# andrew-sha/CUDAFluidSimulator

Measured on AMD Instinct MI355X. Metric: particle-steps/sec (first 41 of the 100 steps of -m time), higher is better.
Workload: dtype f32

## Files before the change

### cudafluidsimulator_amd/csrc/sweep_common.h

```cpp
#pragma once
#include "sph_device.h"

#define SW_THREADS 256
#define SW_WAVES (SW_THREADS / SPH_WAVE)
#ifndef SW_UNROLL
#define SW_UNROLL 4
#endif
#ifndef SW_CAP
#define SW_CAP 384
#endif
#ifndef SW_QCAP
#define SW_QCAP 32
#endif

__device__ __forceinline__ int3 sweep_cell(const DevParams &P, float x, float y,
                                           float z) {
    int3 c;
    c.x = min(max((int)(x / P.h), 0), P.D - 1);
    c.y = min(max((int)(y / P.h), 0), P.D - 1);
    c.z = min(max((int)(z / P.h), 0), P.D - 1);
    return c;
}

__device__ __forceinline__ void load_runs(const DevParams &P,
                                          const int2 *__restrict__ cellRange,
                                          int3 c, bool valid, int (&js)[9],
                                          int (&je)[9]) {
    const int x0 = max(c.x - 1, 0), x1 = min(c.x + 1, P.D - 1);
    const int xm = min(x0 + 1, x1);
    int2 r0[9], r1[9], r2[9];
#pragma unroll
    for (int r = 0; r < 9; ++r) {
        const int sz = min(max(c.z + (r / 3 - 1), 0), P.D - 1);
        const int sy = min(max(c.y + (r % 3 - 1), 0), P.D - 1);
        const int base = sy * P.D + sz * P.D * P.D;
        r0[r] = cellRange[base + x0];
        r1[r] = cellRange[base + xm];
        r2[r] = cellRange[base + x1];
    }
#pragma unroll
    for (int r = 0; r < 9; ++r) {
        const int sz = c.z + (r / 3 - 1), sy = c.y + (r % 3 - 1);
        const bool inGrid = valid && sy >= 0 && sy < P.D && sz >= 0 && sz < P.D;
        const bool n0 = r0[r].y > r0[r].x, n1 = r1[r].y > r1[r].x, n2 = r2[r].y > r2[r].x;
        const bool any = inGrid && (n0 | n1 | n2);
        const int s = n0 ? r0[r].x : (n1 ? r1[r].x : r2[r].x);
        const int e = n2 ? r2[r].y : (n1 ? r1[r].y : r0[r].y);
        js[r] = any ? s : 0;
        je[r] = any ? e : 0;
    }
}


__device__ __forceinline__ void density_pair(const DevParams &P, float pix, float piy,
                                             float piz, float4 pj, float &rho) {
    float dx = pix - pj.x;
    float dy = piy - pj.y;
    float dz = piz - pj.z;
    float dist2 = dx * dx + dy * dy + dz * dz;
    if (!(dist2 > P.h2)) {
        float diff = P.h2 - dist2;
        rho += SPH_MASS * (P.dcoef * diff * diff * diff);
    }
}

struct ForceAcc {
    float fx, fy, fz;
};

__device__ __forceinline__ float sw_recip_refined(float b) {
    const float r0 = __builtin_amdgcn_rcpf(b);
    const float e0 = __builtin_fmaf(-b, r0, 1.0f);
    return __builtin_fmaf(e0, r0, r0);
}
__device__ __forceinline__ float sw_div_with(float a, float b, float r1) {
    const float q0 = a * r1;
    const float e1 = __builtin_fmaf(-b, q0, a);
    const float q1 = __builtin_fmaf(e1, r1, q0);
    const float e2 = __builtin_fmaf(-b, q1, a);
    return __builtin_fmaf(e2, r1, q1);
}
__device__ __forceinline__ float sw_sqrt(float x) {
    const float s = __builtin_amdgcn_sqrtf(x);
    const float sm = __int_as_float(__float_as_int(s) - 1);
    const float sp = __int_as_float(__float_as_int(s) + 1);
    const float tm = __builtin_fmaf(-sm, s, x);
    const float tp = __builtin_fmaf(-sp, s, x);
    float r = (0.f >= tm) ? sm : s;
    r = (0.f < tp) ? sp : r;
    return r;
}

template <bool SLIM>
__device__ __forceinline__ void force_pair(const DevParams &P, float pix, float piy,
                                           float piz, float vix, float viy, float viz,
                                           float prs_i, float4 pj, float4 vj,
                                           ForceAcc &F) {
    float dx = pix - pj.x;
    float dy = piy - pj.y;
    float dz = piz - pj.z;
    float dist2 = dx * dx + dy * dy + dz * dz;
    float rho_j = vj.w;
    float prs_j = fmaxf(0.f, SPH_GAS_CONSTANT * (rho_j - SPH_REST_DENSITY));
    if constexpr (SLIM) {
        const float dist = sw_sqrt(dist2);
        const bool tiny = dist < SPH_EPS_F;
        const bool inP = !(dist2 > P.h2) && !tiny, inV = !(dist > P.h) && !tiny;
        const float rrho = sw_recip_refined(rho_j);
        const float hd = P.h - dist;
        const float fPressure = 0.5f * sw_div_with(-SPH_MASS * (prs_i + prs_j), rho_j, rrho);
        const float scale = sw_div_with((-P.vcoef) * hd * hd, dist, sw_recip_refined(dist));
        const float fViscosity = sw_div_with(SPH_VISCOSITY * SPH_MASS * (P.vcoef * hd), rho_j, rrho);
        const float scaleG = inP ? scale : 0.f, fViscG = inV ? fViscosity : 0.f;
        float kx = dx * scaleG, ky = dy * scaleG, kz = dz * scaleG;
        kx *= fPressure;
        ky *= fPressure;
        kz *= fPressure;
        float dvx = vj.x - vix, dvy = vj.y - viy, dvz = vj.z - viz;
        dvx *= fViscG;
        dvy *= fViscG;
        dvz *= fViscG;
        F.fx += kx;
        F.fy += ky;
        F.fz += kz;
        F.fx += dvx;
        F.fy += dvy;
        F.fz += dvz;
    } else {
        float dist = sqrtf(dist2);
        bool tiny = dist < SPH_EPS_F;
        if (!(dist2 > P.h2) && !tiny) {
            float fPressure = -SPH_MASS * (prs_i + prs_j) / (2.f * rho_j);
            float scale = (-P.vcoef) * (P.h - dist) * (P.h - dist) / dist;
            float kx = dx * scale, ky = dy * scale, kz = dz * scale;
            kx *= fPressure;
            ky *= fPressure;
            kz *= fPressure;
            F.fx += kx;
            F.fy += ky;
            F.fz += kz;
        }
        if (!(dist > P.h) && !tiny) {
            float fViscosity =
                SPH_VISCOSITY * SPH_MASS * (P.vcoef * (P.h - dist)) / rho_j;
            float dvx = vj.x - vix, dvy = vj.y - viy, dvz = vj.z - viz;
            dvx *= fViscosity;
            dvy *= fViscosity;
            dvz *= fViscosity;
            F.fx += dvx;
            F.fy += dvy;
            F.fz += dvz;
        }
    }
}

__device__ __forceinline__ float fast_dist2(float pix, float piy, float piz, float4 pj,
                                            float &dx, float &dy, float &dz) {
    dx = pix - pj.x;
    dy = piy - pj.y;
    dz = piz - pj.z;
    return __builtin_fmaf(dz, dz, __builtin_fmaf(dy, dy, dx * dx));
}

__device__ __forceinline__ void force_pair_fast(const DevParams &P, float pix, float piy,
                                                float piz, float vix, float viy, float viz,
                                                float prs_i, float4 pj, float4 vj,
                                                ForceAcc &F) {
    float dx, dy, dz;
    const float dist2 = fast_dist2(pix, piy, piz, pj, dx, dy, dz);
    const float rho_j = vj.w;
    const float inv_rho = __builtin_amdgcn_rcpf(rho_j);
    const float prs_j = fmaxf(0.f, rho_j - SPH_REST_DENSITY);
    const float inv_dist = __builtin_amdgcn_rsqf(dist2);
    const float dist = dist2 * inv_dist;
    const bool ok = !(dist2 > P.h2) && !(dist < SPH_EPS_F) && dist2 > 0.f;
    if (ok) {
        const float hd = P.h - dist;
        const float s = (0.5f * SPH_MASS * P.vcoef) * (prs_i + prs_j) * inv_rho * (hd * hd) * inv_dist;
        const float fv = (SPH_VISCOSITY * SPH_MASS * P.vcoef) * hd * inv_rho;
        F.fx = __builtin_fmaf(vj.x - vix, fv, __builtin_fmaf(dx, s, F.fx));
        F.fy = __builtin_fmaf(vj.y - viy, fv, __builtin_fmaf(dy, s, F.fy));
        F.fz = __builtin_fmaf(vj.z - viz, fv, __builtin_fmaf(dz, s, F.fz));
    }
}

__device__ __forceinline__ void integrate_particle(const DevParams &P, float4 &p,
                                                   float &vx, float &vy, float &vz,
                                                   const ForceAcc &F, float density) {
    const float timestep = P.dt;
    vx += timestep * F.fx / density;
    vy += timestep * (F.fy / density + SPH_GRAVITY);
    vz += timestep * F.fz / density;

    p.x += timestep * vx;
    p.y += timestep * vy;
    p.z += timestep * vz;

    if (p.x < P.h) { p.x = P.h; vx *= -SPH_ELASTICITY; }
    else if (p.x > P.boxHi) { p.x = P.boxHi; vx *= -SPH_ELASTICITY; }
    if (p.y < P.h) { p.y = P.h; vy *= -SPH_ELASTICITY; }
    else if (p.y > P.boxHi) { p.y = P.boxHi; vy *= -SPH_ELASTICITY; }
    if (p.z < P.h) { p.z = P.h; vz *= -SPH_ELASTICITY; }
    else if (p.z > P.boxHi) { p.z = P.boxHi; vz *= -SPH_ELASTICITY; }

    if (fabsf(vx) < SPH_EPS_F) vx = 0;
    if (fabsf(vy) < SPH_EPS_F) vy = 0;
    if (fabsf(vz) < SPH_EPS_F) vz = 0;
}

__device__ __forceinline__ void store_particle(const SweepArgs &A, int i, float4 p,
                                               float vx, float vy, float vz,
                                               float rho, const ForceAcc &F) {
    A.pos_out[i] = p;
    A.vel_out[i] = make_float4(vx, vy, vz, rho);
    if (A.host_order_pos) {
        uint32_t id = __float_as_uint(p.w);
        float *o = A.host_order_pos + 3 * (size_t)id;
        o[0] = p.x;
        o[1] = p.y;
        o[2] = p.z;
    }
    if (A.force_out) A.force_out[i] = make_float4(F.fx, F.fy, F.fz, 0.f);
}

__device__ __forceinline__ int xcd_tile(int b, int nb, int C, int rot = 0) {
    int base = 0, R = nb, r = b;
    if (C > 0) {
        const int G = 8 * C;
        const int ng = nb / G, g = b / G;
        if (g < ng) {
            r = b - g * G;
            const int x = rot > 0 ? ((r & 7) + g / rot) & 7 : (r & 7);
            return g * G + x * C + (r >> 3);
        }
        base = ng * G;
        R = nb - base;
        r = b - base;
    }
    const int xcd = r & 7, idx = r >> 3;
    const int q = R >> 3, rem = R & 7;
    return base + xcd * q + min(xcd, rem) + idx;
}

__device__ __forceinline__ uint32_t wave_sum_u32(uint32_t v) {
#pragma unroll
    for (int off = 32; off > 0; off >>= 1) v += __shfl_xor(v, off);
    return v;
}
```

### cudafluidsimulator_amd/csrc/sweeps_list.hip

```cpp
#include "sweep_common.h"

#define SL_NONE 0xFFFFFFFFu

#ifndef SL_WINDOW
#define SL_WINDOW 160
#endif
#ifndef SL_K1_THREADS
#define SL_K1_THREADS 64
#endif

#ifndef SL_K1_WAVES
#define SL_K1_WAVES 6
#endif
__device__ __forceinline__ void sl_store_quiet(const SweepArgs &A, int i, bool valid, float rho, int lane) {
    const unsigned long long calm = A.calm[(i - lane) >> 6];
    const float prs = fmaxf(0.f, SPH_GAS_CONSTANT * (rho - SPH_REST_DENSITY));
    const bool q = valid && prs == 0.f && ((calm >> lane) & 1ull);
    const unsigned long long qb = __ballot(q), vb = __ballot(valid);
    if (lane == 0) {
        reinterpret_cast<unsigned long long *>(A.quiet)[(i - lane) >> 6] = qb;
        if (A.quietAll && qb != vb) *A.quietAll = 0u;
    }
}
__device__ __forceinline__ uint32_t sl_quiet_window(const uint32_t *__restrict__ quiet, uint32_t j) {
    const uint32_t lo = quiet[j >> 5], hi = quiet[(j >> 5) + 1];
    return __builtin_amdgcn_alignbit(hi, lo, j & 31u);
}

__device__ __forceinline__ int wave_max_i32(int v) {
#pragma unroll
    for (int off = 32; off > 0; off >>= 1) v = max(v, __shfl_xor(v, off));
    return v;
}

template <bool FAST, bool SAMECUT>
__global__ __launch_bounds__(SL_K1_THREADS, SL_K1_WAVES * SL_K1_THREADS / 64)
void k_density_mask_lds(DevParams P, SweepArgs A) {
    __shared__ float4 stageAll[SL_K1_THREADS / SPH_WAVE][SW_CAP + SW_UNROLL];
    const int lane = threadIdx.x & 63, w = threadIdx.x >> 6;
    float4 *stage = stageAll[w];
    const int wv = xcd_tile(blockIdx.x, gridDim.x, A.tileChunk * (256 / SL_K1_THREADS), A.tileRotate) * (SL_K1_THREADS / SPH_WAVE) + w;
    const int i = A.i_origin + wv * SPH_WAVE + lane;
    const bool valid = i >= A.i_begin && i < A.i_end;
    const bool anyValid = __ballot(valid) != 0ull;
    float4 pi = valid ? A.pos4[i] : make_float4(0, 0, 0, 0);
    int3 c = sweep_cell(P, pi.x, pi.y, pi.z);
    int js[9], je[9];
    load_runs(P, A.cellRange, c, valid, js, je);

    int words = 0;
    uint32_t pairs = 0;
#pragma unroll
    for (int r = 0; r < 9; ++r) {
        words += (je[r] - js[r] + 31) >> 5;
        pairs += (uint32_t)(je[r] - js[r]);
    }
    const int Q = __builtin_amdgcn_readfirstlane((wave_max_i32(words) + 1) >> 1);
    const int shard = wv & (SL_POOL_SHARDS - 1);
    unsigned long long base = 0;
    if (lane == 0) base = atomicAdd(A.maskCursor + shard * SL_CURSOR_STRIDE, (unsigned long long)Q * SPH_WAVE);
    base = (unsigned long long)__builtin_amdgcn_readfirstlane((unsigned)(base >> 32)) << 32 |
           (unsigned long long)__builtin_amdgcn_readfirstlane((unsigned)base);
    const unsigned long long subCap = A.maskCapacity / SL_POOL_SHARDS;
    const bool ok = base + (unsigned long long)Q * SPH_WAVE <= subCap;
    base += (unsigned long long)shard * subCap;
    if (lane == 0 && anyValid) {
        A.maskOff[2 * (size_t)wv] = ok ? (uint32_t)base : SL_NONE;
        A.maskOff[2 * (size_t)wv + 1] = (uint32_t)Q;
        if (!ok) A.noneList[atomicAdd(A.maskCursor + 1, 1ull)] = (uint32_t)wv;
    }
    uint4 *const myq = reinterpret_cast<uint4 *>(A.maskPool) + (ok ? base : 0ull) + lane;
    if (A.pairCounter) {
        uint32_t s = wave_sum_u32(pairs);
        if (lane == 0) atomicAdd(A.pairCounter + 16 + (wv & 255) * 16, (unsigned long long)s);
    }

    if (lane < SW_UNROLL) stage[SW_CAP + lane] = make_float4(1e18f, 1e18f, 1e18f, 0.f);
    const float4 *const sent = stage + SW_CAP;
    float rho = 0.f;
    float h2v = P.h2, dcv = P.dcoef, cut2r = P.cut2, massv = SPH_MASS;
    asm volatile("" : "+v"(h2v), "+v"(dcv), "+v"(cut2r), "+v"(massv));
    uint32_t pj0 = 0, pm0 = 0;
    bool pending = false;
    int qidx = 0;
    uint32_t hcount = 0;
    auto emit = [&](uint32_t jbase, uint32_t mask) {
        if (ok && mask != 0) {
            hcount += (uint32_t)__builtin_popcount(mask);
            if (!pending) {
                pj0 = jbase;
                pm0 = mask;
                pending = true;
            } else {
                myq[(size_t)qidx * SPH_WAVE] = make_uint4(pj0, pm0, jbase, mask);
                ++qidx;
                pending = false;
            }
        }
    };
    const int rowId = c.y + c.z * P.D;
    unsigned long long todo = __ballot(valid);
    bool unify = false;
    if (todo) {
        const int row0 = __builtin_amdgcn_readlane(rowId, __ffsll((long long)todo) - 1);
        if (__ballot(valid && rowId != row0)) {
            unify = true;
#pragma unroll
            for (int r = 0; r < 9; ++r) {
                const unsigned long long mm = __ballot(valid && je[r] > js[r]);
                if (mm) {
                    const int u0 = __builtin_amdgcn_readlane(js[r], __ffsll((long long)mm) - 1);
                    const int u1 = __builtin_amdgcn_readlane(je[r], 63 - __clzll((long long)mm));
                    unify = unify && (u1 - u0) <= SW_CAP;
                }
            }
        }
    }
    struct Run {
        int jsr, len, u0, ulen;
        bool any, staged;
    };
    auto describe = [&](int r, bool act) -> Run {
        int jsr = js[0], jer = je[0];
#pragma unroll
        for (int q = 1; q < 9; ++q) {
            jsr = (r == q) ? js[q] : jsr;
            jer = (r == q) ? je[q] : jer;
        }
        Run R;
        const bool nonempty = act && jer > jsr;
        const unsigned long long mm = __ballot(nonempty);
        R.any = mm != 0;
        const int lo = mm ? __ffsll((long long)mm) - 1 : 0;
        const int hi = mm ? 63 - __clzll((long long)mm) : 0;
        R.u0 = __builtin_amdgcn_readlane(jsr, lo);
        R.ulen = R.any ? __builtin_amdgcn_readlane(jer, hi) - R.u0 : 0;
        R.staged = R.ulen <= SW_CAP;
        R.jsr = nonempty ? jsr : R.u0;
        R.len = nonempty ? jer - jsr : 0;
        return R;
    };
    while (todo) {
        const int leader = __ffsll((long long)todo) - 1;
        const int rowL = __builtin_amdgcn_readlane(rowId, leader);
        const bool act = valid && (unify || rowId == rowL);
        todo &= ~__ballot(act);
#pragma unroll 1
        for (int r = 0; r < 9; ++r) {
            const Run R = describe(r, act);
            if (R.any && R.staged) {
                for (int k = lane; k < R.ulen; k += SPH_WAVE) stage[k] = A.pos4[R.u0 + k];
                __builtin_amdgcn_fence(__ATOMIC_RELEASE, "wavefront");
                __builtin_amdgcn_wave_barrier();
            }
            if (R.any) {
                const int jsr = R.jsr, len = R.len;
                const float4 *cur = stage + (jsr - R.u0);
                const float4 *gcur = A.pos4 + jsr;
                uint32_t m = 0;
                int k = 0;
                auto trip = [&](const float4 (&pj)[SW_UNROLL]) {
#pragma unroll
                    for (int u = 0; u < SW_UNROLL; ++u) {
                        float dx = pi.x - pj[u].x;
                        float dy = pi.y - pj[u].y;
                        float dz = pi.z - pj[u].z;
                        float dist2;
                        float draw;
                        if (FAST) {
                            dist2 = __builtin_fmaf(dz, dz, __builtin_fmaf(dy, dy, dx * dx));
                            draw = h2v - dist2;
                            const float diff = fmaxf(draw, 0.f);
                            rho = __builtin_fmaf((massv * dcv) * (diff * diff), diff, rho);
                        } else {
                            dist2 = dx * dx + dy * dy + dz * dz;
                            draw = h2v - dist2;
                            float diff;
                            asm("v_max_f32_e32 %0, 0, %1" : "=v"(diff) : "v"(draw));
                            rho += massv * (dcv * diff * diff * diff);
                        }
                        if (SAMECUT) {
                            m = __builtin_amdgcn_alignbit(m, __float_as_uint(draw), 31);
                            continue;
                        }
                        asm("v_cmp_ngt_f32_e32 vcc, %1, %2\n\tv_addc_co_u32_e32 %0, vcc, %0, %0, vcc"
                            : "+v"(m)
                            : "v"(dist2), "v"(cut2r)
                            : "vcc");
                    }
#pragma unroll
                    for (int u = 0; u < SW_UNROLL; ++u) asm volatile("" ::"v"(pj[u].w));
                    if (((k + SW_UNROLL) & 31) == 0) {
                        if (SAMECUT) emit((uint32_t)(jsr + (k & ~31)), ~__builtin_bitreverse32(m));
                        else emit((uint32_t)(jsr + (k & ~31)), __builtin_bitreverse32(m));
                        m = 0;
                    }
                };
                if (R.staged) {
                    for (; __ballot(k < len); k += SW_UNROLL) {
                        float4 pj[SW_UNROLL];
#pragma unroll
                        for (int u = 0; u < SW_UNROLL; ++u) {
                            const float4 *p = (k + u < len) ? cur + k : sent;
                            pj[u] = p[u];
                        }
                        trip(pj);
                    }
                } else {
                    for (; __ballot(k < len); k += SW_UNROLL) {
                        float4 pj[SW_UNROLL];
#pragma unroll
                        for (int u = 0; u < SW_UNROLL; ++u) {
                            const bool in = k + u < len;
                            pj[u] = gcur[in ? k + u : 0];
                            pj[u].x = in ? pj[u].x : 1e18f;
                        }
                        trip(pj);
                    }
                }
                if ((k & 31) != 0) {
                    if (SAMECUT) emit((uint32_t)(jsr + (k & ~31)), (~__builtin_bitreverse32(m)) >> (32 - (k & 31)));
                    else emit((uint32_t)(jsr + (k & ~31)), __builtin_bitreverse32(m) >> (32 - (k & 31)));
                }
                __builtin_amdgcn_fence(__ATOMIC_ACQUIRE, "wavefront");
                __builtin_amdgcn_wave_barrier();
            }
        }
    }
    if (ok && valid) {
        if (pending) myq[(size_t)qidx * SPH_WAVE] = make_uint4(pj0, pm0, 0u, 0u);
        else if (qidx < Q) myq[(size_t)qidx * SPH_WAVE] = make_uint4(0u, 0u, 0u, 0u);
    }
    if (valid) {
        rho = fmaxf(rho, SPH_EPS_F);
        if (A.rhoToVel4) A.vel4[i].w = rho;
        A.pv8[2 * (size_t)i + 1].w = rho;
    }
    if (A.quiet) sl_store_quiet(A, i, valid, rho, lane);
    if (A.hitCount && valid) A.hitCount[i] = hcount;
}

#ifndef SL_SORT_SHIFT
#define SL_SORT_SHIFT 3
#endif
#define SL_DEAL_THREADS 256
#define SL_DEAL_ROWS SL_DEAL_THREADS
#define SL_DEAL_WINDOW (SL_DEAL_ROWS + SL_WINDOW - SPH_WAVE)
static_assert(SL_WINDOW >= SPH_WAVE, "the dealt sweep needs the window");

template <bool FAST, bool SLIM>
__global__ __launch_bounds__(SL_DEAL_THREADS) void k_force_dealt(DevParams P, SweepArgs A) {
    __shared__ uint32_t sortBase[128];
    __shared__ uint16_t rowOf[SL_DEAL_ROWS];
    __shared__ float4 win[2 * SL_DEAL_WINDOW];
    const int t = threadIdx.x, lane = t & 63;
    const bool second = (int)blockIdx.x >= A.nblk1;
    const int rb = second ? A.i_begin2 : A.i_begin, re = second ? A.i_end2 : A.i_end;
    const int chunk = A.tileChunk > 0 ? max(A.tileChunk * 256 / SL_DEAL_ROWS, 1) : 0;
    const int group = ((rb - A.i_origin) >> 6) / (SL_DEAL_ROWS / SPH_WAVE) +
                      xcd_tile(second ? (int)blockIdx.x - A.nblk1 : (int)blockIdx.x,
                               second ? (int)gridDim.x - A.nblk1 : A.nblk1, chunk, A.tileRotate);
    const int R0 = A.i_origin + group * SL_DEAL_ROWS;
    const unsigned long long *const quiet64 = reinterpret_cast<const unsigned long long *>(A.quiet);

    unsigned long long qw = 0ull;
    bool inPlace = false;
    if (A.quiet) {
        const int r0 = R0 + (t & ~63);
        const int lo = max(rb - r0, 0), hi = min(re - r0, 64);
        const unsigned long long vm = hi > lo ? ((hi - lo == 64 ? ~0ull : (1ull << (hi - lo)) - 1ull) << lo) : 0ull;
        if (vm) qw = quiet64[r0 >> 6];
        inPlace = __syncthreads_and((qw & vm) == vm) != 0;
    }
    if (!inPlace) {
        for (int b = t; b < 128; b += SL_DEAL_THREADS) sortBase[b] = 0u;
        __syncthreads();
        const int row = R0 + t;
        const bool counted = row >= rb && row < re && !((qw >> lane) & 1ull);
        const uint32_t bucket = min((counted ? A.hitCount[row] : 0u) >> SL_SORT_SHIFT, 127u);
        const uint32_t slot = atomicAdd(&sortBase[bucket], 1u);
        __syncthreads();
        if (t < SPH_WAVE) {
            const uint32_t a = sortBase[2 * t], b = sortBase[2 * t + 1];
            uint32_t incl = a + b;
#pragma unroll
            for (int off = 1; off < SPH_WAVE; off <<= 1) {
                const uint32_t up = __shfl_up(incl, off);
                incl += t >= off ? up : 0u;
            }
            const uint32_t excl = incl - (a + b);
            sortBase[2 * t] = excl;
            sortBase[2 * t + 1] = excl + a;
        }
        __syncthreads();
        rowOf[sortBase[bucket] + slot] = (uint16_t)t;
    }

    const bool allQuiet = A.quietAll && __builtin_amdgcn_readfirstlane(*A.quietAll) != 0u &&
                          (!A.quietHalo || __builtin_amdgcn_readfirstlane(*A.quietHalo) != 0u);
    const int w0 = max(R0 - (SL_WINDOW - SPH_WAVE) / 2, 0);
    int wlen = max(min(SL_DEAL_WINDOW, A.n_all - w0), 0);
    {
        bool wanted = !allQuiet && wlen > 0;
        if (wanted && A.quiet) {
            const int k0 = w0 >> 6, k1 = (w0 + wlen - 1) >> 6;
            wanted = k0 + t <= k1 && quiet64[k0 + t] != ~0ull;
        }
        if (__syncthreads_or(wanted)) {
            for (int k = t; k < 2 * wlen; k += SL_DEAL_THREADS) win[k] = A.pv8[2 * (size_t)w0 + k];
            __syncthreads();
        } else {
            wlen = 0;
        }
    }

    {
        const int i = R0 + (inPlace ? t : (int)rowOf[t]);
        const bool inRange = i >= rb && i < re;
        const int iSafe = inRange ? i : rb;
        float4 pi = A.pv8[2 * (size_t)iSafe];
        const float4 vi = A.pv8[2 * (size_t)iSafe + 1];
        const float prs_i = fmaxf(0.f, SPH_GAS_CONSTANT * (vi.w - SPH_REST_DENSITY));
        const int rel = iSafe - A.i_origin;
        const uint32_t baseq = inRange ? A.maskOff[2 * (size_t)(rel >> 6)] : SL_NONE;
        const int Q = inRange ? (int)A.maskOff[2 * (size_t)(rel >> 6) + 1] : 0;
        const bool valid = inRange && baseq != SL_NONE;
        ForceAcc F = {0.f, 0.f, 0.f};
        if (!allQuiet) {
            const uint4 *const sbase = reinterpret_cast<const uint4 *>(A.maskPool);
            const uint32_t send = valid ? baseq + (uint32_t)Q * SPH_WAVE : 0u;
            uint32_t sidx = valid ? baseq + (uint32_t)(rel & 63) : 0u;
            uint32_t m = 0, mq[2] = {0u, 0u};
            int jb = 0, jq[2] = {0, 0};
            bool live = true;
            const bool qi = A.quiet && valid && ((A.quiet[i >> 5] >> (i & 31)) & 1u);
            auto fetch = [&]() {
                while (sidx < send) {
                    uint4 q = sbase[sidx];
                    sidx = (q.w == 0u) ? send : sidx + SPH_WAVE;
                    if (qi) {
                        q.y &= ~sl_quiet_window(A.quiet, q.x);
                        q.w &= ~sl_quiet_window(A.quiet, q.z);
                    }
                    if (q.y == 0u) {
                        q.x = q.z;
                        q.y = q.w;
                        q.w = 0u;
                    }
                    jq[0] = (int)q.x;
                    mq[0] = q.y;
                    jq[1] = (int)q.z;
                    mq[1] = q.w;
                    if (q.y != 0u) break;
                }
            };
            fetch();
            if (__ballot(mq[0] != 0u)) {
                auto pop = [&]() -> int {
                    if (m == 0) {
                        m = mq[0];
                        jb = jq[0];
                        mq[0] = mq[1];
                        jq[0] = jq[1];
                        mq[1] = 0;
                        if (mq[0] == 0) fetch();
                    }
                    live = (m | mq[0]) != 0;
                    const bool has = m != 0;
                    const int b = has ? __builtin_ctz(m) : 0;
                    m &= m - 1u;
                    return has ? jb + b : iSafe;
                };
                auto body = [&](const float4 &pj, const float4 &vj) {
                    if (FAST) force_pair_fast(P, pi.x, pi.y, pi.z, vi.x, vi.y, vi.z, prs_i, pj, vj, F);
                    else force_pair<SLIM>(P, pi.x, pi.y, pi.z, vi.x, vi.y, vi.z, prs_i, pj, vj, F);
                };
#define SD_UNDEF4(q) asm volatile("" : "=v"(q.x), "=v"(q.y), "=v"(q.z), "=v"(q.w));
#define SD_FETCH(j, p, v)                                                      \
    SD_UNDEF4(p)                                                               \
    SD_UNDEF4(v)                                                               \
    if ((unsigned)((j)-w0) >= (unsigned)wlen) {                                \
        p = A.pv8[2 * (size_t)(j)];                                            \
        v = A.pv8[2 * (size_t)(j) + 1];                                        \
    }
#define SD_USE(j, p, v)                                                        \
    if ((unsigned)((j)-w0) < (unsigned)wlen) {                                 \
        p = win[2 * ((j)-w0)];                                                 \
        v = win[2 * ((j)-w0) + 1];                                             \
    }                                                                          \
    body(p, v);
                float4 p0 = make_float4(0, 0, 0, 0), v0 = p0, p1 = p0, v1 = p0;
                int j0 = pop();
                SD_FETCH(j0, p0, v0)
                int j1 = pop();
                SD_FETCH(j1, p1, v1)
                for (;;) {
                    SD_USE(j0, p0, v0)
                    if (!__ballot(live)) { SD_USE(j1, p1, v1) break; }
                    j0 = pop();
                    SD_FETCH(j0, p0, v0)
                    SD_USE(j1, p1, v1)
                    if (!__ballot(live)) { SD_USE(j0, p0, v0) break; }
                    j1 = pop();
                    SD_FETCH(j1, p1, v1)
                }
#undef SD_FETCH
#undef SD_USE
#undef SD_UNDEF4
            }
        }
        if (valid) {
            float vx = vi.x, vy = vi.y, vz = vi.z;
            integrate_particle(P, pi, vx, vy, vz, F, vi.w);
            store_particle(A, i, pi, vx, vy, vz, vi.w, F);
        }
    }
}

__global__ __launch_bounds__(256) void k_halo_quiet(const float4 *__restrict__ pv8, int lo_end, int hi_begin, int n_all,
                                                    const float4 *__restrict__ vref, const uint32_t *__restrict__ ownedQuiet,
                                                    uint32_t *__restrict__ haloQuiet) {
    if (*ownedQuiet == 0u) return;
    const int t = blockIdx.x * blockDim.x + threadIdx.x;
    if (t >= lo_end + (n_all - hi_begin)) return;
    const int j = t < lo_end ? t : hi_begin + (t - lo_end);
    const float4 v = pv8[2 * (size_t)j + 1], r = *vref;
    const float prs = fmaxf(0.f, SPH_GAS_CONSTANT * (v.w - SPH_REST_DENSITY));
    if (!(prs == 0.f && v.x == r.x && v.y == r.y && v.z == r.z)) *haloQuiet = 0u;
}
void sph_launch_halo_quiet(const float4 *pv8, int lo_end, int hi_begin, int n_all, const float4 *vref,
                           const uint32_t *ownedQuiet, uint32_t *haloQuiet, hipStream_t s) {
    const int rows = lo_end + (n_all - hi_begin);
    if (rows > 0) k_halo_quiet<<<(rows + 255) / 256, 256, 0, s>>>(pv8, lo_end, hi_begin, n_all, vref, ownedQuiet, haloQuiet);
}

__global__ __launch_bounds__(256) void k_count_hits(SweepArgs A) {
    const int i = A.i_begin + blockIdx.x * blockDim.x + threadIdx.x;
    uint32_t n = 0, dropped = 0;
    if (i < A.i_end) {
        const int wv = (i - A.i_origin) >> 6;
        const uint32_t baseq = A.maskOff[2 * (size_t)wv];
        const int Q = (int)A.maskOff[2 * (size_t)wv + 1];
        if (baseq != SL_NONE) {
            const uint4 *q4 = reinterpret_cast<const uint4 *>(A.maskPool) + baseq + (threadIdx.x & 63);
            const bool qi = A.quiet && ((A.quiet[i >> 5] >> (i & 31)) & 1u);
            for (int q = 0; q < Q; ++q) {
                const uint4 t = q4[(size_t)q * SPH_WAVE];
                n += (uint32_t)__builtin_popcount(t.y) + (uint32_t)__builtin_popcount(t.w);
                if (qi)
                    dropped += (uint32_t)__builtin_popcount(t.y & sl_quiet_window(A.quiet, t.x)) +
                               (uint32_t)__builtin_popcount(t.w & sl_quiet_window(A.quiet, t.z));
                if (t.w == 0u) break;
            }
        }
    }
    n = wave_sum_u32(n);
    dropped = wave_sum_u32(dropped);
    if ((threadIdx.x & 63) == 0 && n) {
        atomicAdd(A.pairCounter + 16 + (blockIdx.x & 255) * 16 + 15, (unsigned long long)n);
        atomicAdd(A.pairCounter + 16 + (blockIdx.x & 255) * 16 + 14, (unsigned long long)(n - dropped));
    }
}

void sph_launch_density_list(const DevParams &P, const SweepArgs &A, int mathMode, hipStream_t s) {
    int cnt = A.i_end - A.i_begin;
    if (cnt <= 0) return;
    int blocks = (A.i_end - A.i_origin + SL_K1_THREADS - 1) / SL_K1_THREADS;
    const bool same = P.cut2 == P.h2;
    if (mathMode == 1) {
        if (same) k_density_mask_lds<true, true><<<blocks, SL_K1_THREADS, 0, s>>>(P, A);
        else k_density_mask_lds<true, false><<<blocks, SL_K1_THREADS, 0, s>>>(P, A);
    } else {
        if (same) k_density_mask_lds<false, true><<<blocks, SL_K1_THREADS, 0, s>>>(P, A);
        else k_density_mask_lds<false, false><<<blocks, SL_K1_THREADS, 0, s>>>(P, A);
    }
    if (A.pairCounter) k_count_hits<<<(cnt + 255) / 256, 256, 0, s>>>(A);
}

#define SL_FALLBACK_BLOCKS 512
template <bool FAST, bool SLIM>
__global__ __launch_bounds__(SPH_WAVE) void k_force_fallback(DevParams P, SweepArgs A) {
    const unsigned count = (unsigned)A.maskCursor[1];
    for (unsigned idx = blockIdx.x; idx < count; idx += gridDim.x) {
    const int i = A.i_origin + (int)A.noneList[idx] * SPH_WAVE + (int)threadIdx.x;
    const bool mine = (i >= A.i_begin && i < A.i_end) || (i >= A.i_begin2 && i < A.i_end2);
    if (!__ballot(mine)) continue;
    const int iSafe = mine ? i : A.i_begin;
    float4 pi = A.pv8[2 * (size_t)iSafe];
    const float4 vi = A.pv8[2 * (size_t)iSafe + 1];
    const float prs_i = fmaxf(0.f, SPH_GAS_CONSTANT * (vi.w - SPH_REST_DENSITY));
    int3 c = sweep_cell(P, pi.x, pi.y, pi.z);
    int js[9], je[9];
    load_runs(P, A.cellRange, c, mine, js, je);
    ForceAcc F = {0.f, 0.f, 0.f};
#pragma unroll
    for (int r = 0; r < 9; ++r)
        for (int j = js[r]; j < je[r]; ++j) {
            if (FAST) force_pair_fast(P, pi.x, pi.y, pi.z, vi.x, vi.y, vi.z, prs_i, A.pv8[2 * (size_t)j], A.pv8[2 * (size_t)j + 1], F);
            else force_pair<SLIM>(P, pi.x, pi.y, pi.z, vi.x, vi.y, vi.z, prs_i, A.pv8[2 * (size_t)j], A.pv8[2 * (size_t)j + 1], F);
        }
    if (mine) {
        float vx = vi.x, vy = vi.y, vz = vi.z;
        integrate_particle(P, pi, vx, vy, vz, F, vi.w);
        store_particle(A, i, pi, vx, vy, vz, vi.w, F);
    }
    }
}

__global__ void k_patch_pv8(const float4 *__restrict__ vel4, float4 *__restrict__ pv8, int i_begin,
                            int i_end, int n_all) {
    int t = blockIdx.x * blockDim.x + threadIdx.x;
    int j = t < i_begin ? t : i_end + (t - i_begin);
    if (j < n_all) pv8[2 * (size_t)j + 1] = vel4[j];
}

void sph_launch_patch_halo(const SweepArgs &A, hipStream_t s) {
    const int halo = A.i_begin + (A.n_all - A.i_end);
    if (halo > 0) k_patch_pv8<<<(halo + 255) / 256, 256, 0, s>>>(A.vel4, A.pv8, A.i_begin, A.i_end, A.n_all);
}

void sph_launch_force_list(const DevParams &P, const SweepArgs &A, int mathMode, hipStream_t s) {
    SweepArgs B = A;
    if (B.i_end2 <= B.i_begin2) B.i_begin2 = B.i_end2 = 0;
    if (B.i_end <= B.i_begin) {
        B.i_begin = B.i_begin2;
        B.i_end = B.i_end2;
        B.i_begin2 = B.i_end2 = 0;
    }
    if (B.i_end <= B.i_begin) return;
    if (B.patchHalo) sph_launch_patch_halo(B, s);
    const int wpb = SL_DEAL_ROWS / SPH_WAVE, threads = SL_DEAL_THREADS;
    auto blocks_of = [&](int a, int b) {
        if (b <= a) return 0;
        const int w0 = (a - B.i_origin) >> 6, w1 = (b - B.i_origin + 63) >> 6;
        return (w1 + wpb - 1) / wpb - w0 / wpb;
    };
    B.nblk1 = blocks_of(B.i_begin, B.i_end);
    const int fblocks = B.nblk1 + blocks_of(B.i_begin2, B.i_end2);
    const int blocks = SL_FALLBACK_BLOCKS;
    if (mathMode == 1) {
        k_force_dealt<true, true><<<fblocks, threads, 0, s>>>(P, B);
        k_force_fallback<true, true><<<blocks, SPH_WAVE, 0, s>>>(P, B);
    } else if (P.slimDiv) {
        k_force_dealt<false, true><<<fblocks, threads, 0, s>>>(P, B);
        k_force_fallback<false, true><<<blocks, SPH_WAVE, 0, s>>>(P, B);
    } else {
        k_force_dealt<false, false><<<fblocks, threads, 0, s>>>(P, B);
        k_force_fallback<false, false><<<blocks, SPH_WAVE, 0, s>>>(P, B);
    }
}
```

Measured before the change: 4.510 billion.

## Add per-run SoA LDS ring staging for distinct neighbor cell runs in list sweep

Adds a ring-buffer path for the neighbor-list sweep that is taken when a wave covers only a few distinct cell runs (at most SW_RING_SLOTS). Each distinct run is loaded in chunks of 64 particles into its own LDS slot in structure-of-arrays form, so lanes can read x, y and z for four neighbors with three vector loads. The aim is to avoid staging the whole union range with per-neighbor float4 loads, and to let lanes in different rows share the stage even when their ranges are disjoint. The cost is extra ballots, readlanes and wave barriers per chunk, plus padded lanes that compute against sentinel positions when runs have uneven lengths.

```diff
diff --git a/cudafluidsimulator_amd/csrc/sweep_common.h b/cudafluidsimulator_amd/csrc/sweep_common.h
--- a/cudafluidsimulator_amd/csrc/sweep_common.h
+++ b/cudafluidsimulator_amd/csrc/sweep_common.h
@@ -9,6 +9,20 @@
 #ifndef SW_CAP
 #define SW_CAP 384
 #endif
+#ifndef SW_RING_SLOTS
+#define SW_RING_SLOTS 4
+#endif
+#ifndef SW_RING_C
+#define SW_RING_C 64
+#endif
+#define SW_RING_G (SW_RING_C <= 32 ? 2 : 1)
+#ifndef SW_RING_BATCH
+#define SW_RING_BATCH 2
+#endif
+#define SW_RING_STRIDE ((3 * SW_RING_C / 4) % 2 ? 3 * SW_RING_C : 3 * SW_RING_C + 4)
+static_assert(SW_RING_C % SW_UNROLL == 0 && SW_RING_C <= 64 / SW_RING_G, "ring chunk: whole trips, one load per lane");
+static_assert(SW_RING_SLOTS % (SW_RING_BATCH * SW_RING_G) == 0 && SW_RING_SLOTS <= 16, "ring slots: whole batches");
+static_assert(SW_RING_SLOTS * SW_RING_STRIDE <= 4 * SW_CAP, "the ring must fit below the slice's sentinel");
 #ifndef SW_QCAP
 #define SW_QCAP 32
 #endif
diff --git a/cudafluidsimulator_amd/csrc/sweeps_list.hip b/cudafluidsimulator_amd/csrc/sweeps_list.hip
--- a/cudafluidsimulator_amd/csrc/sweeps_list.hip
+++ b/cudafluidsimulator_amd/csrc/sweeps_list.hip
@@ -117,8 +117,9 @@
         }
     }
     struct Run {
-        int jsr, len, u0, ulen;
-        bool any, staged;
+        int jsr, len, u0, ulen, slot, nd;
+        unsigned long long starts;
+        bool any, ring, staged;
     };
     auto describe = [&](int r, bool act) -> Run {
         int jsr = js[0], jer = je[0];
@@ -135,6 +136,15 @@
         const int hi = mm ? 63 - __clzll((long long)mm) : 0;
         R.u0 = __builtin_amdgcn_readlane(jsr, lo);
         R.ulen = R.any ? __builtin_amdgcn_readlane(jer, hi) - R.u0 : 0;
+        const int prevS = __shfl_up(jsr, 1), prevE = __shfl_up(jer, 1);
+        const bool prevIn = lane > 0 && ((mm >> (lane - 1)) & 1ull);
+        const bool opens = nonempty && !(prevIn && prevS == jsr && prevE == jer);
+        R.starts = __ballot(opens);
+        R.nd = __builtin_popcountll(R.starts);
+        const int below = (int)__builtin_amdgcn_mbcnt_hi((uint32_t)(R.starts >> 32),
+                                                         __builtin_amdgcn_mbcnt_lo((uint32_t)R.starts, 0u));
+        R.slot = nonempty ? below - (opens ? 0 : 1) : 0;
+        R.ring = R.nd <= SW_RING_SLOTS;
         R.staged = R.ulen <= SW_CAP;
         R.jsr = nonempty ? jsr : R.u0;
         R.len = nonempty ? jer - jsr : 0;
@@ -148,7 +158,7 @@
 #pragma unroll 1
         for (int r = 0; r < 9; ++r) {
             const Run R = describe(r, act);
-            if (R.any && R.staged) {
+            if (R.any && !R.ring && R.staged) {
                 for (int k = lane; k < R.ulen; k += SPH_WAVE) stage[k] = A.pos4[R.u0 + k];
                 __builtin_amdgcn_fence(__ATOMIC_RELEASE, "wavefront");
                 __builtin_amdgcn_wave_barrier();
@@ -159,12 +169,13 @@
                 const float4 *gcur = A.pos4 + jsr;
                 uint32_t m = 0;
                 int k = 0;
-                auto trip = [&](const float4 (&pj)[SW_UNROLL]) {
+                auto trip = [&](const float (&cx)[SW_UNROLL], const float (&cy)[SW_UNROLL],
+                                const float (&cz)[SW_UNROLL], float qx, float qy, float qz) {
 #pragma unroll
                     for (int u = 0; u < SW_UNROLL; ++u) {
-                        float dx = pi.x - pj[u].x;
-                        float dy = pi.y - pj[u].y;
-                        float dz = pi.z - pj[u].z;
+                        float dx = qx - cx[u];
+                        float dy = qy - cy[u];
+                        float dz = qz - cz[u];
                         float dist2;
                         float draw;
                         if (FAST) {
@@ -188,15 +199,77 @@
                             : "v"(dist2), "v"(cut2r)
                             : "vcc");
                     }
-#pragma unroll
-                    for (int u = 0; u < SW_UNROLL; ++u) asm volatile("" ::"v"(pj[u].w));
                     if (((k + SW_UNROLL) & 31) == 0) {
                         if (SAMECUT) emit((uint32_t)(jsr + (k & ~31)), ~__builtin_bitreverse32(m));
                         else emit((uint32_t)(jsr + (k & ~31)), __builtin_bitreverse32(m));
                         m = 0;
                     }
                 };
-                if (R.staged) {
+                auto trip4 = [&](const float4 (&pj)[SW_UNROLL]) {
+                    float cx[SW_UNROLL], cy[SW_UNROLL], cz[SW_UNROLL];
+#pragma unroll
+                    for (int u = 0; u < SW_UNROLL; ++u) {
+                        cx[u] = pj[u].x;
+                        cy[u] = pj[u].y;
+                        cz[u] = pj[u].z;
+                    }
+                    trip(cx, cy, cz, pi.x, pi.y, pi.z);
+#pragma unroll
+                    for (int u = 0; u < SW_UNROLL; ++u) asm volatile("" ::"v"(pj[u].w));
+                };
+                if (R.ring) {
+                    const bool mine = len > 0;
+                    const float qx = mine ? pi.x : -1e18f, qy = mine ? pi.y : -1e18f, qz = mine ? pi.z : -1e18f;
+                    float *const ring = reinterpret_cast<float *>(stage);
+                    const float *const rd = ring + R.slot * SW_RING_STRIDE;
+                    constexpr int L = SPH_WAVE / SW_RING_G;
+                    const int sub = lane / L, idx = lane % L;
+                    while (__ballot(k < len)) {
+                        unsigned long long bits = R.starts;
+                        for (int e = 0; e < R.nd; e += SW_RING_BATCH * SW_RING_G) {
+                            float4 v[SW_RING_BATCH];
+#pragma unroll
+                            for (int b = 0; b < SW_RING_BATCH; ++b) {
+                                int st = 0, ln = 0;
+#pragma unroll
+                                for (int g = 0; g < SW_RING_G; ++g) {
+                                    const int from = bits ? __ffsll((long long)bits) - 1 : 0;
+                                    const int s0 = __builtin_amdgcn_readlane(R.jsr, from);
+                                    const int l0 = bits ? __builtin_amdgcn_readlane(len, from) : 0;
+                                    bits &= bits - 1;
+                                    st = (sub == g) ? s0 : st;
+                                    ln = (sub == g) ? l0 : ln;
+                                }
+                                v[b] = make_float4(1e18f, 1e18f, 1e18f, 0.f);
+                                if (idx < SW_RING_C && k + idx < ln) v[b] = A.pos4[st + k + idx];
+                            }
+#pragma unroll
+                            for (int b = 0; b < SW_RING_BATCH; ++b) {
+                                if (idx < SW_RING_C) {
+                                    float *const dst = ring + (e + b * SW_RING_G + sub) * SW_RING_STRIDE + idx;
+                                    dst[0] = v[b].x;
+                                    dst[SW_RING_C] = v[b].y;
+                                    dst[2 * SW_RING_C] = v[b].z;
+                                }
+                            }
+                        }
+                        __builtin_amdgcn_fence(__ATOMIC_RELEASE, "wavefront");
+                        __builtin_amdgcn_wave_barrier();
+                        const int kc = k;
+                        do {
+                            const float4 x4 = *reinterpret_cast<const float4 *>(rd + (k - kc));
+                            const float4 y4 = *reinterpret_cast<const float4 *>(rd + SW_RING_C + (k - kc));
+                            const float4 z4 = *reinterpret_cast<const float4 *>(rd + 2 * SW_RING_C + (k - kc));
+                            const float cx[SW_UNROLL] = {x4.x, x4.y, x4.z, x4.w};
+                            const float cy[SW_UNROLL] = {y4.x, y4.y, y4.z, y4.w};
+                            const float cz[SW_UNROLL] = {z4.x, z4.y, z4.z, z4.w};
+                            trip(cx, cy, cz, qx, qy, qz);
+                            k += SW_UNROLL;
+                        } while (k - kc < SW_RING_C && __ballot(k < len));
+                        __builtin_amdgcn_fence(__ATOMIC_ACQUIRE, "wavefront");
+                        __builtin_amdgcn_wave_barrier();
+                    }
+                } else if (R.staged) {
                     for (; __ballot(k < len); k += SW_UNROLL) {
                         float4 pj[SW_UNROLL];
 #pragma unroll
@@ -204,7 +277,7 @@
                             const float4 *p = (k + u < len) ? cur + k : sent;
                             pj[u] = p[u];
                         }
-                        trip(pj);
+                        trip4(pj);
                     }
                 } else {
                     for (; __ballot(k < len); k += SW_UNROLL) {
@@ -215,7 +288,7 @@
                             pj[u] = gcur[in ? k + u : 0];
                             pj[u].x = in ? pj[u].x : 1e18f;
                         }
-                        trip(pj);
+                        trip4(pj);
                     }
                 }
                 if ((k & 31) != 0) {
```

Result: no change. 4.441 billion, median of 2 (-1.5%).
